# UoL-SignalProcessingGroup/SMC-NUTS

Hardware: NVIDIA B200
Metric: leapfrog_grad_evals_per_s (higher is better)
Workload: dtype f64

## Files before the change

### include/smcnuts_b200.h

```cpp
#ifndef SMCNUTS_B200_H
#define SMCNUTS_B200_H

#include <stdint.h>

#ifdef __cplusplus
extern "C" {
#endif

#define SMCB_MODEL_ARMA 0
#define SMCB_MODEL_PRMWCD 1
#define SMCB_MODEL_GAUSS 2

#define SMCB_STREAM_NUTS 0
#define SMCB_STREAM_MOMENTUM 1
#define SMCB_STREAM_ACCREJ 2
#define SMCB_STREAM_RESAMPLE 3
#define SMCB_STREAM_INIT 4
#define SMCB_STREAM_ESTIMATE 5

#define SMCB_CONSTRAIN_NONE 0
#define SMCB_CONSTRAIN_EXP_LAST 1

int smcb_version(void);
int smcb_build_flavour(void);
const char* smcb_last_error(void);
long long smcb_launch_count(void);

int smcb_model_create(int kind, const double* host_data, long long n, int dim, void** handle);
int smcb_model_create_plugin(const char* so_path, const double* host_data, long long n, void** handle);
int smcb_model_set_scale(void* handle, const double* host_scale);
int smcb_model_destroy(void* handle);
int smcb_model_dim(void* handle);
int smcb_model_constrained_dim(void* handle);
int smcb_model_constrain(void* handle, const double* x, long long N, double* out, void* stream);
int smcb_debug_pack_prm(const double* host_scalar_blob, int n_obs, int tiles, double* host_out, long long n_out);

int smcb_logp_grad(void* handle, const double* x, long long N, double phi, double* A, double* B, double* grad,
                   void* stream);
int smcb_combine_logp(const double* A, const double* B, double phi, long long N, double* out, void* stream);

int smcb_nuts_workspace_bytes(void* handle, long long N, int max_depth, long long* bytes);
int smcb_nuts_set_blocks_per_sm(int blocks_per_sm);
int smcb_nuts_transition(void* handle, const double* x, const double* r, long long N, double eps, double phi,
                         int max_depth, int accrej, uint64_t seed, uint32_t iteration, uint64_t particle0,
                         double* x_new, double* r_new, double* A_old, double* B_old, double* A_new, double* B_new,
                         double* ke_old, double* ke_new, int* n_leapfrog, int* accepted, int* depth, double* accept_stat,
                         const double* A_in, const double* B_in, const double* g_in, double* g_new, void* workspace,
                         long long workspace_bytes, void* stream);

int smcb_normals(uint64_t seed, uint32_t iteration, uint32_t stream_id, uint64_t particle0, long long N, int D,
                 double* out, void* stream);
int smcb_uniforms(uint64_t seed, uint32_t iteration, uint32_t stream_id, uint64_t particle0, long long N,
                  uint32_t draw, double* out, void* stream);

int smcb_row_half_sqnorm(const double* r, long long N, int D, double* out, void* stream);
int smcb_std_normal_logpdf(const double* x, long long N, int D, double* out, void* stream);
int smcb_uniform_logw(const double* logZ, long long N_total, long long N, double* out, void* stream);
int smcb_affine(const double* in, long long N, double a, double b, double* out, void* stream);
int smcb_init_logw(const double* lp, const double* x, long long N, int D, double* logw, void* stream);
int smcb_reweight_forward(const double* logw, const double* lp_x, const double* lp_xnew, const double* r,
                          const double* r_new, long long N, int D, double* out, void* stream);
int smcb_reweight_forward_ke(const double* logw, const double* lp_x, const double* lp_xnew, const double* ke_old,
                             const double* ke_new, long long N, double* out, void* stream);
int smcb_reweight_forward_split(const double* logw, const double* A_old, const double* B_old, const double* A_new,
                                const double* B_new, const double* ke_old, const double* ke_new, double phi, long long N,
                                double* out, void* stream);
int smcb_reweight_general(const double* logw, const double* lp_x, const double* lp_xnew, const double* L,
                          const double* q, long long N, double* out, void* stream);
int smcb_reweight_asymptotic(const double* logw, const double* A, const double* B, double phi_new, double phi_old,
                             long long N, double* out, void* stream);

long long smcb_reduce_workspace_bytes(void);
int smcb_lse_partial(const double* logw, long long N, double* out3, void* workspace, void* stream);
int smcb_lse_finalize(const double* triples, int P, double* out2, void* stream);
int smcb_normalise(const double* logw, long long N, const double* logZ, double* wn, void* stream);

int smcb_tempering_arrays(const double* A, const double* B, double phi_old, long long N, double* logpri,
                          double* loglik, double* c, void* stream);
int smcb_ess_multi_phi(const double* loglik, const double* logpri, const double* c, long long N,
                       const double* phis, int m, double* out, void* workspace, void* stream);

long long smcb_bisect_state_bytes(void);
int smcb_bisect_max_candidates(void);
int smcb_bisect_passes(void);
int smcb_bisect_init(void* state, double xa, double xb, double target, void* stream);
int smcb_bisect_eval(const double* A, const double* B, double phi_old, long long N, const void* state, double* out,
                     void* workspace, void* stream);
int smcb_bisect_step(const double* triples, int P, void* state, void* stream);
int smcb_bisect_read(const void* state, double* out4, void* stream);

long long smcb_scan_workspace_bytes(long long N);
int smcb_cdf(const double* wn, long long N, const double* offset_in, const double* total_in, double* cdf,
             double* total_out, void* workspace, void* stream);
int smcb_normalise_tilesums(const double* logw, long long N, const double* logZ, double* wn, double* total_out,
                            void* workspace, void* stream);
int smcb_cdf_from_tilesums(const double* wn, long long N, const double* offset_total, double* cdf, void* workspace,
                           void* stream);
int smcb_ancestors_multinomial(const double* cdf, long long N, const double* u, long long M, int64_t* idx,
                               void* stream);
int smcb_ancestors_systematic(const double* cdf, long long N, double u0, long long j0, long long M_total,
                              long long M, int64_t* idx, void* stream);
long long smcb_resample_workspace_bytes(long long M, int D);
int smcb_resample_systematic(const double* cdf, long long N, double u0, const double* u0_dev, long long j0,
                             long long M_total, long long M, const double* x, int D, double* out, int64_t* idx,
                             void* workspace, void* stream);
int smcb_resample_systematic_push(const double* cdf, long long N, double u0, long long j0, long long M_total,
                                  long long M, const double* x, int D, double* const* peer_out, long long rows_per_rank,
                                  int64_t* idx, void* workspace, void* stream);
int smcb_resample_multinomial_push(const double* cdf, long long n, const double* ends, int rank, int P, uint64_t seed,
                                   uint32_t iteration, uint32_t stream_id, long long N_total, long long particle0,
                                   const double* x, int D, double* const* peer_out, int64_t* const* peer_idx,
                                   long long rows_per_rank, void* stream);
int smcb_rank_offsets(const double* totals, int P, int rank, double* out2, void* stream);
int smcb_peer_alloc(long long bytes, void** ptr, void* handle64);
int smcb_peer_open(const void* handle64, void** ptr);
int smcb_peer_close(void* ptr);
int smcb_peer_free(void* ptr);
int smcb_gather_rows(const double* x, const int64_t* idx, long long M, int D, double* out, void* stream);

int smcb_scale_rows(const double* x, long long N, int D, const double* scale, int inverse, double* out, void* stream);

int smcb_weighted_moment(const double* x, const double* wn, long long N, int D, int constrain, const double* center,
                         int power, double* out, void* workspace, void* stream);
int smcb_weighted_moments12(const double* x, const double* wn, long long N, int D, int constrain, const double* center,
                            double* out2D, void* workspace, void* stream);
int smcb_moments12_finalize(const double* sums2D, const double* center, int D, double* mean, double* var, void* stream);
int smcb_count_moved(const double* x, const double* x_new, long long N, int D, double* out_count, void* workspace,
                     void* stream);

int smcb_gaussL_sums(const double* r_new, const double* x_new, long long N, int D, double* sums, void* stream);
int smcb_gaussL_gram(const double* r_new, const double* x_new, long long N, int D, const double* mean, double* gram,
// ... 23 lines not shown
```

### smc-nuts_b200/csrc/capi.cuh

```cuda
#pragma once
#include <cuda_runtime.h>

#include <atomic>
#include <cstdio>
#include <string>

#include "../../include/smcnuts_b200.h"
#include "common.cuh"
#include "models.cuh"

namespace smcb {

#if defined(SMCB_PLUGIN_TU)
inline std::string& last_error_ref() {
    static thread_local std::string s;
    return s;
}
inline std::atomic<long long> g_launches{0};
#else
std::string& last_error_ref();
extern std::atomic<long long> g_launches;
#endif

inline int fail(const char* where, const char* what) {
    last_error_ref() = std::string(where) + ": " + what;
    return -1;
}
inline int check_launch(const char* where) {
    g_launches.fetch_add(1, std::memory_order_relaxed);
    cudaError_t e = cudaGetLastError();
    if (e != cudaSuccess) return fail(where, cudaGetErrorString(e));
    return 0;
}
#define SMCB_CUDA(call)                                                        \
    do {                                                                       \
        cudaError_t e_ = (call);                                               \
        if (e_ != cudaSuccess) return ::smcb::fail(#call, cudaGetErrorString(e_)); \
    } while (0)
#define SMCB_REQUIRE(cond, msg)                          \
    do {                                                 \
        if (!(cond)) return ::smcb::fail(__func__, msg); \
    } while (0)

#define SMCB_PLUGIN_ABI 2
struct NutsArgs;
struct PluginVT {
    void* dl;
    int (*abi)(void);
    int (*dim)(void);
    int (*ndata)(void);
    const char* (*last_error)(void);
    long long (*nuts_workspace_bytes)(const ModelDesc*, long long, int);
    int (*nuts_transition)(const ModelDesc*, const NutsArgs*, long long, void*);
    int (*logp_grad)(const ModelDesc*, const double*, long long, double, double*, double*, double*, void*);
    int (*constrained_dim)(void);
    int (*constrain)(const ModelDesc*, const double*, long long, double*, void*);
};

struct Model {
    ModelDesc desc;
    double* d_data;
    PluginVT* vt = nullptr;
    double* d_scale = nullptr;
};

#if defined(SMCB_PLUGIN_TU)
inline int device_sm_count() {
    static int n = 0;
    if (!n) {
        int dev = 0;
        cudaGetDevice(&dev);
        cudaDeviceGetAttribute(&n, cudaDevAttrMultiProcessorCount, dev);
        if (n <= 0) n = 148;
    }
    return n;
}
#else
int device_sm_count();
#endif

inline int stride_grid(long long n, int threads, int per_sm) {
    long long want = (n + threads - 1) / threads;
    long long cap = (long long)device_sm_count() * per_sm;
    if (want < 1) want = 1;
    return (int)(want < cap ? want : cap);
}

}
```

### smc-nuts_b200/csrc/nuts_kernel.cu

```cuda
#include <dlfcn.h>

#include <cstdlib>
#include <cstring>
#include <vector>

#include "nuts_builtin.cuh"

namespace smcb {

std::string& last_error_ref() {
    static thread_local std::string s;
    return s;
}
std::atomic<long long> g_launches{0};
static thread_local int g_nuts_blocks_per_sm = 0;

int device_sm_count() {
    static int n = 0;
    if (!n) {
        int dev = 0;
        cudaGetDevice(&dev);
        cudaDeviceGetAttribute(&n, cudaDevAttrMultiProcessorCount, dev);
        if (n <= 0) n = 148;
    }
// ... 152 lines not shown
    if (N == 0) return 0;
    const Model* m = (const Model*)handle;
    if (m->vt->constrain(&m->desc, x, N, out, stream)) return fail("smcb_model_constrain (plug-in)", m->vt->last_error());
    g_launches.fetch_add(1, std::memory_order_relaxed);
    return 0;
}

int smcb_debug_pack_prm(const double* host_scalar_blob, int n_obs, int tiles, double* host_out, long long n_out) {
    SMCB_REQUIRE(host_scalar_blob && host_out && n_obs > 0 && tiles > 0 && n_obs <= 8 * tiles, "bad argument");
    SMCB_REQUIRE(n_out >= 32 + (long long)tiles * 9 * 32, "output too small: 32 + tiles * 288 doubles");
    pack_prm_fragments(host_scalar_blob, n_obs, tiles, host_out);
    return 0;
}

int smcb_logp_grad(void* handle, const double* x, long long N, double phi, double* A, double* B, double* grad,
                   void* stream) {
    SMCB_REQUIRE(handle && x && N >= 0, "bad argument");
    if (N == 0) return 0;
    const Model* m = (const Model*)handle;
    cudaStream_t st = (cudaStream_t)stream;
    if (m->vt) {
        if (m->vt->logp_grad(&m->desc, x, N, phi, A, B, grad, stream)) return fail("smcb_logp_grad (plug-in)", m->vt->last_error());
        g_launches.fetch_add(1, std::memory_order_relaxed);
        return 0;
    }
    switch (m->desc.kind) {
        case kArma: return launch_logp<ArmaModel>(m, x, N, phi, A, B, grad, st);
        case kPRMwCD: return launch_logp<PrmModel>(m, x, N, phi, A, B, grad, st);
        default: return launch_logp<GaussModel>(m, x, N, phi, A, B, grad, st);
    }
}

int smcb_combine_logp(const double* A, const double* B, double phi, long long N, double* out, void* stream) {
    SMCB_REQUIRE(A && B && out && N >= 0, "bad argument");
    if (N == 0) return 0;
    combine_logp_kernel<<<stride_grid(N, 256, 8), 256, 0, (cudaStream_t)stream>>>(A, B, phi, N, out);
    return check_launch("combine_logp_kernel");
}

int smcb_nuts_set_blocks_per_sm(int blocks_per_sm) {
    SMCB_REQUIRE(blocks_per_sm >= 0, "blocks_per_sm must be >= 0 (0 = as many as fit)");
    g_nuts_blocks_per_sm = blocks_per_sm;
    return 0;
}

int smcb_nuts_workspace_bytes(void* handle, long long N, int max_depth, long long* bytes) {
    SMCB_REQUIRE(handle && bytes && N >= 0, "bad argument");
    SMCB_REQUIRE(max_depth >= 1 && max_depth <= 10, "max_depth must be in [1, 10] (reference: MAX_TREE_DEPTH = 10)");
    const Model* m = (const Model*)handle;
    long long b;
    if (m->vt) {
        b = m->vt->nuts_workspace_bytes(&m->desc, N, max_depth);
        if (b < 0) return fail("smcb_nuts_workspace_bytes (plug-in)", "occupancy query failed");
        *bytes = b;
        return 0;
    }
    if (m->desc.scale) {
        b = nuts_ws_bytes_scaled(m, N, max_depth);
        if (b < 0) return fail("smcb_nuts_workspace_bytes", "occupancy query failed");
        *bytes = b;
        return 0;
    }
    switch (m->desc.kind) {
        case kArma: b = nuts_ws_bytes<ArmaModel>(m, N, max_depth); break;
        case kPRMwCD:
            b = prm_use_group(m->desc, N) ? nuts_ws_bytes<PrmModelG<kPrmTiles>>(m, N, max_depth) : nuts_ws_bytes<PrmModel>(m, N, max_depth);
            break;
        default: {
#define WS_G(K) nuts_ws_bytes<GaussModelG<K>>(m, N, max_depth)
            b = SMCB_GAUSS_DISPATCH(m->desc.dim, WS_G, nuts_ws_bytes<GaussModel>(m, N, max_depth));
#undef WS_G
            break;
        }
    }
    if (b < 0) return fail("smcb_nuts_workspace_bytes", "occupancy query failed");
    *bytes = b;
    return 0;
}

int smcb_nuts_transition(void* handle, const double* x, const double* r, long long N, double eps, double phi,
                         int max_depth, int accrej, uint64_t seed, uint32_t iteration, uint64_t particle0,
                         double* x_new, double* r_new, double* A_old, double* B_old, double* A_new, double* B_new,
                         double* ke_old, double* ke_new, int* n_leapfrog, int* accepted, int* depth, double* accept_stat,
                         const double* A_in, const double* B_in, const double* g_in, double* g_new, void* workspace,
                         long long workspace_bytes, void* stream) {
    SMCB_REQUIRE(handle && x && r && x_new && r_new && workspace, "null argument");
    SMCB_REQUIRE((A_in && B_in && g_in) || (!A_in && !B_in && !g_in), "A_in, B_in, g_in: all three or none");
    SMCB_REQUIRE(!(accrej && (g_in || g_new)), "gradient carry-over is not available with the accept-reject epilogue");
    SMCB_REQUIRE(g_new != x_new && (!g_in || (g_in != g_new)), "g_new must not alias its inputs");
    SMCB_REQUIRE(x != x_new && r != r_new, "x_new/r_new must not alias x/r");
    SMCB_REQUIRE(max_depth >= 1 && max_depth <= 10, "max_depth must be in [1, 10] (reference: MAX_TREE_DEPTH = 10)");
    SMCB_REQUIRE(iteration < (1u << 24), "iteration must be < 2^24");
    if (N <= 0) return N == 0 ? 0 : fail("smcb_nuts_transition", "negative N");
    const Model* m = (const Model*)handle;
    NutsArgs a{};
    a.model = m->desc;
    a.x = x; a.r = r; a.N = N; a.eps = eps; a.phi = phi; a.max_depth = max_depth; a.accrej = accrej;
    a.seed = seed; a.iteration = iteration; a.particle0 = particle0;
    a.x_new = x_new; a.r_new = r_new; a.A_old = A_old; a.B_old = B_old; a.A_new = A_new; a.B_new = B_new;
    a.ke_old = ke_old; a.ke_new = ke_new; a.n_leapfrog = n_leapfrog; a.accepted = accepted; a.depth = depth;
    a.accept_stat = accept_stat;
    a.blocks_per_sm = g_nuts_blocks_per_sm;
    a.A_in = A_in; a.B_in = B_in; a.g_in = g_in; a.g_new = g_new;
    a.ws = (double*)workspace;
    cudaStream_t st = (cudaStream_t)stream;
    if (m->vt) {
        if (m->vt->nuts_transition(&m->desc, &a, workspace_bytes, stream)) return fail("smcb_nuts_transition (plug-in)", m->vt->last_error());
        g_launches.fetch_add(1, std::memory_order_relaxed);
        return 0;
    }
    if (m->desc.scale) return launch_nuts_scaled(m, a, workspace_bytes, st);
    switch (m->desc.kind) {
        case kArma: return launch_nuts<ArmaModel>(m, a, workspace_bytes, st);
        case kPRMwCD:
            return prm_use_group(m->desc, N) ? launch_nuts<PrmModelG<kPrmTiles>>(m, a, workspace_bytes, st)
                                          : launch_nuts<PrmModel>(m, a, workspace_bytes, st);
        default: {
#define LAUNCH_G(K) launch_nuts<GaussModelG<K>>(m, a, workspace_bytes, st)
            return SMCB_GAUSS_DISPATCH(m->desc.dim, LAUNCH_G, launch_nuts<GaussModel>(m, a, workspace_bytes, st));
#undef LAUNCH_G
        }
    }
}

}
```

### smc-nuts_b200/csrc/nuts_lane.cuh

```cuda
#pragma once
#include "common.cuh"
#include "models.cuh"
#include "philox.cuh"

namespace smcb {

struct NutsArgs {
    ModelDesc model;
    const double* x;
    const double* r;
    long long N;
    double eps, phi;
    int max_depth;
    int accrej;
    uint64_t seed;
    uint32_t iteration;
    uint64_t particle0;
    double* x_new;
    double* r_new;
    double* A_old;
    double* B_old;
    double* A_new;
    double* B_new;
    double* ke_old;
    double* ke_new;
    int* n_leapfrog;
    int* accepted;
    int* depth;
    double* accept_stat;
    const double* A_in;
    const double* B_in;
    const double* g_in;
    double* g_new;
    double* ws;
    unsigned long long* queue;
    void* exchange;
    int blocks_per_sm;
};

struct alignas(16) D2 {
    double x, y;
};

SMCB_HD int nuts_nlp(int nl) { return (nl + 1) & ~1; }
SMCB_HD int nuts_stage_stride(int nl) { return 2 * nuts_nlp(nl) + 2; }
SMCB_HD int nuts_slot_stride(int nl, bool carry) { return 2 * nuts_nlp(nl) + 2 + (carry ? nuts_nlp(nl) : 0); }
constexpr int kNutsHdr = 8;
SMCB_HD int nuts_ws_doubles(int nl, int L, bool carry = true) {
    return ((kNutsHdr + 3 * nuts_nlp(nl) + nuts_slot_stride(nl, carry) * (2 * L + 3)) + 15) & ~15;
}

enum LanePhase : int { kIdle = 0, kInit = 1, kLeaf = 2 };

template <class M>
struct Lane {
    static constexpr int G = M::GROUP;
    static constexpr int DM = M::NLOC;
    double xa[DM], ra[DM], ga[DM];
    double logu;
    long long pid;
    double* ws;
    double* stg;
    int nlp_, slot_stride;
    int phase, dir, depth, D, L, nl, sub;
    uint32_t leaf, n_tot, n_leapfrog;
    uint32_t ck_used, cand_used, ck_valid;
    uint32_t samp_used;
    int samp_ref;
    uint64_t pend_n, pend_ref, ck_ref;
    StreamReader rng;

#define SMCB_LOCAL(i) for (int i = 0; i < (M::STATIC_NL ? M::STATIC_NL : nl); ++i)
#define SMCB_PAIRS(i) for (int i = 0; i < (M::STATIC_NL ? M::STATIC_NL : nl); i += 2)

    SMCB_HD int gd(int i) const { return G == 1 ? i : sub + G * i; }
    SMCB_HD uint64_t draw_bits(const NutsArgs& a) {
        return rng.next_bits(a.seed, (a.iteration << 8) | (uint32_t)kStreamNuts, a.particle0 + (uint64_t)pid);
    }
    SMCB_HD double draw(const NutsArgs& a) { return (double)draw_bits(a) * 0x1.0p-53; }
    SMCB_HD bool draw_below_ratio(const NutsArgs& a, uint32_t num, uint32_t den) {
        const uint64_t k = draw_bits(a);
        return k * (uint64_t)den < ((uint64_t)num << 53);
    }
    SMCB_HD int nlp_get() const { return M::STATIC_NL ? ((M::STATIC_NL + 1) & ~1) : nlp_; }
#define nlp nlp_get()
    SMCB_HD double gsum(double v) const {
#if defined(SMCB_WARP_CODE)
        if (G > 1) {
            const unsigned mask = ((1u << G) - 1u) << ((threadIdx.x & 31u) & ~(unsigned)(G - 1));
#pragma unroll
            for (int o = 1; o < G; o <<= 1) v += __shfl_xor_sync(mask, v, o);
        }
#endif
        return v;
    }

#ifndef SMCB_WIDE_RECORDS_CG
#define SMCB_WIDE_RECORDS_CG 1
#endif
    static constexpr bool kCg = (SMCB_WIDE_RECORDS_CG != 0) && M::STAGE;
// ... 488 lines not shown
```

### smc-nuts_b200/csrc/nuts_launch.cuh

```cuda
#pragma once
#include <cstdlib>

#include "capi.cuh"
#include "nuts_lane.cuh"

namespace smcb {

inline int blocks_per_sm_cap(int requested) {
    if (requested > 0) return requested;
    const char* e = getenv("SMCB_NUTS_BLOCKS_PER_SM");
    const int v = e ? atoi(e) : 0;
    return v > 0 ? v : 1 << 20;
}

template <class M> struct LaunchCfg { static constexpr int NT = 256, MIN_BLOCKS = 1; };

#ifndef SMCB_ALIGN_PARITY
#define SMCB_ALIGN_PARITY 0
#endif
template <class M> struct AlignCfg { static constexpr bool ON = (SMCB_ALIGN_PARITY != 0) && M::GROUP > 1; };

template <class M>
static size_t nuts_smem_bytes(const ModelDesc& d) {
    size_t n = (size_t)M::staged_doubles(d);
    if (M::STAGE) n += (size_t)LaunchCfg<M>::NT * nuts_stage_stride(M::STATIC_NL);
    return sizeof(double) * n;
}

template <class M> struct StageOffset { static int of(const ModelDesc&) { return 0; } };
template <class M> struct LaunchCfg<ScaledModel<M>> : LaunchCfg<M> {};
template <class M> struct StageOffset<ScaledModel<M>> : StageOffset<M> {};


template <class M>
__device__ __forceinline__ const double* stage_model(const ModelDesc& d, double* smem, int staged, int offset) {
    if constexpr (M::STATIC_NL != 0) {
        for (int i = threadIdx.x; i < staged; i += blockDim.x) smem[i] = d.data[offset + i];
        __syncthreads();
        return smem;
    } else {
        return d.data;
    }
}

#ifndef SMCB_TAIL_COMPACT
#define SMCB_TAIL_COMPACT 1
#endif
template <class M> struct TailCfg {
    static constexpr bool ON = (SMCB_TAIL_COMPACT != 0) && M::GROUP == 1 && !M::STAGE && !AlignCfg<M>::ON;
};

template <class M>
static size_t nuts_exchange_bytes(long long blocks) {
    return TailCfg<M>::ON ? (size_t)blocks * LaunchCfg<M>::NT * sizeof(Lane<M>) : 0;
}

template <class M>
__global__ void __launch_bounds__(LaunchCfg<M>::NT, LaunchCfg<M>::MIN_BLOCKS)
nuts_transition_kernel(NutsArgs a, int staged, int stage_offset, int rec_doubles) {
    extern __shared__ double smem[];
    constexpr int G = M::GROUP;
    constexpr int NW = LaunchCfg<M>::NT / 32;
    __shared__ int s_tail;
    __shared__ int s_cnt[2][NW];
    if (threadIdx.x == 0) s_tail = 0;
    M model(a.model, stage_model<M>(a.model, smem, staged, stage_offset));
    if constexpr (TailCfg<M>::ON) __syncthreads();
    const unsigned lane_id = threadIdx.x & 31u;
    Lane<M> lane;
    lane.idle_init(model, (int)(lane_id % G));
    lane.stg = M::STAGE ? smem + staged + (size_t)threadIdx.x * nuts_stage_stride(M::STATIC_NL) : nullptr;
    double* ws = a.ws + (size_t)(blockIdx.x * blockDim.x + threadIdx.x) * rec_doubles;
    constexpr unsigned kLeaders = G == 1 ? 0xffffffffu : 0x11111111u;
    const unsigned group_first = lane_id & ~(unsigned)(G - 1);
    bool drained = false;
    const unsigned admit_parity = a.g_in ? 1u : 0u;
    bool reported = false;
    for (unsigned trip = 0;; ++trip) {
        if constexpr (TailCfg<M>::ON) {
            if (*(volatile int*)&s_tail == NW) break;
        }
        const bool admit = !AlignCfg<M>::ON || ((trip & 1u) == admit_parity);
        const bool want = (lane.phase == kIdle) && !drained && admit;
        const unsigned m = __ballot_sync(0xffffffffu, want) & kLeaders;
        if (m) {
            const int leader = __ffs(m) - 1;
            unsigned long long base = 0;
            if ((int)lane_id == leader) base = atomicAdd(a.queue, (unsigned long long)__popc(m));
            base = __shfl_sync(0xffffffffu, base, leader);
            if (want) {
                const long long p = (long long)base + __popc(m & ((1u << group_first) - 1u));
                if (p < a.N) lane.begin(a, model, p, ws);
                else drained = true;
            }
            if constexpr (TailCfg<M>::ON) {
                if (!reported && __any_sync(0xffffffffu, drained)) {
                    if (lane_id == 0) atomicAdd(&s_tail, 1);
                    reported = true;
                }
            }
        }
        if (__all_sync(0xffffffffu, lane.phase == kIdle)) {
            if (!AlignCfg<M>::ON || __all_sync(0xffffffffu, drained)) break;
            continue;
        }
        if (lane.phase != kIdle) { lane.pre_eval(a); lane.prefetch_ck(); }
        double A, B, g[M::NLOC];
        if constexpr (G > 1) __syncwarp();
        model.eval(lane.xa, a.phi, A, B, g);
        lane.take_grad(g);
        if (lane.phase != kIdle) lane.post_eval(a, A, B);
    }
    if constexpr (TailCfg<M>::ON) {
        Lane<M>* exch = reinterpret_cast<Lane<M>*>(a.exchange) + (size_t)blockIdx.x * blockDim.x;
        const int warp = threadIdx.x >> 5;
        constexpr int kPerWarp = 32 / G;
        for (unsigned trip = 0;; ++trip) {
            const bool act = lane.phase != kIdle;
            const unsigned b = __ballot_sync(0xffffffffu, act) & kLeaders;
            if (lane_id == 0) s_cnt[trip & 1u][warp] = __popc(b);
            __syncthreads();
            int total = 0, before = 0, have = 0;
#pragma unroll
            for (int w = 0; w < NW; ++w) {
                const int c = s_cnt[trip & 1u][w];
                total += c;
                before += (w < warp) ? c : 0;
                have += (c > 0) ? 1 : 0;
            }
            if (total == 0) break;
            if (have > (total + kPerWarp - 1) / kPerWarp) {
                if (act) exch[(before + __popc(b & ((1u << group_first) - 1u))) * G + lane.sub] = lane;
                __threadfence();
                __syncthreads();
                if ((int)threadIdx.x < total * G) {
                    double* const stg = lane.stg;
                    lane = exch[threadIdx.x];
                    lane.stg = stg;
                } else {
                    lane.phase = kIdle;
                }
            }
            if (__all_sync(0xffffffffu, lane.phase == kIdle)) continue;
            if (lane.phase != kIdle) { lane.pre_eval(a); lane.prefetch_ck(); }
            double A, B, g[M::NLOC];
            if constexpr (G > 1) __syncwarp();
            model.eval(lane.xa, a.phi, A, B, g);
            lane.take_grad(g);
            if (lane.phase != kIdle) lane.post_eval(a, A, B);
        }
    }
}

template <class M>
__global__ void __launch_bounds__(128) logp_grad_kernel(ModelDesc md, const double* __restrict__ x, long long N,
                                                        double phi, double* __restrict__ Aout,
                                                        double* __restrict__ Bout, double* __restrict__ grad,
                                                        int staged) {
    extern __shared__ double smem[];
    M model(md, stage_model<M>(md, smem, staged, 0));
    const int D = M::STATIC_D ? M::STATIC_D : model.dim();
    for (long long i = blockIdx.x * (long long)blockDim.x + threadIdx.x; i < N; i += (long long)gridDim.x * blockDim.x) {
        double xv[M::DMAX], g[M::DMAX], A, B;
#pragma unroll
        for (int d = 0; d < (M::STATIC_D ? M::STATIC_D : D); ++d) xv[d] = x[i * D + d];
        model.eval(xv, phi, A, B, g);
        if (Aout) Aout[i] = A;
        if (Bout) Bout[i] = B;
        if (grad) {
            const bool bad = !is_finite(A + phi * B);
#pragma unroll
            for (int d = 0; d < (M::STATIC_D ? M::STATIC_D : D); ++d) grad[i * D + d] = bad ? neg_inf() : g[d];
        }
    }
}


template <class M>
static long long nuts_blocks(const Model* mdl, long long N, size_t smem, int* occ_out, int requested = 0) {
    const int NT = LaunchCfg<M>::NT;
    auto kern = nuts_transition_kernel<M>;
    if (smem > 48 * 1024) cudaFuncSetAttribute(kern, cudaFuncAttributeMaxDynamicSharedMemorySize, (int)smem);
    int occ = 0;
    if (cudaOccupancyMaxActiveBlocksPerMultiprocessor(&occ, kern, NT, smem) != cudaSuccess || occ < 1) return -1;
    if (occ > blocks_per_sm_cap(requested)) occ = blocks_per_sm_cap(requested);
    long long blocks = (long long)device_sm_count() * occ;
    const long long need = (N * M::GROUP + NT - 1) / NT;
    if (blocks > need) blocks = need;
    if (blocks < 1) blocks = 1;
    if (occ_out) *occ_out = occ;
    (void)mdl;
    return blocks;
}

template <class M>
static long long nuts_ws_bytes(const Model* mdl, long long N, int max_depth) {
    const size_t smem = nuts_smem_bytes<M>(mdl->desc);
    const long long blocks = nuts_blocks<M>(mdl, N, smem, nullptr);
    if (blocks < 0) return -1;
    M probe(mdl->desc, nullptr);
    return (long long)sizeof(double) * nuts_ws_doubles(probe.nloc(), max_depth) * blocks * LaunchCfg<M>::NT + 256 +
           (long long)nuts_exchange_bytes<M>(blocks);
}

template <class M>
static int launch_nuts(const Model* mdl, NutsArgs a, long long ws_bytes, cudaStream_t st) {
    const int NT = LaunchCfg<M>::NT;
    const int staged = M::staged_doubles(mdl->desc);
    const size_t smem = nuts_smem_bytes<M>(mdl->desc);
    const long long blocks = nuts_blocks<M>(mdl, a.N, smem, nullptr, a.blocks_per_sm);
    if (blocks < 0) return fail("smcb_nuts_transition", "kernel does not fit on an SM");
    M probe(mdl->desc, nullptr);
    const int rec = nuts_ws_doubles(probe.nloc(), a.max_depth, a.g_new != nullptr);
    const long long rec_bytes = (long long)sizeof(double) * rec * blocks * NT;
    const long long ws_need = rec_bytes + 256 + (long long)nuts_exchange_bytes<M>(blocks);
    if (ws_bytes < ws_need) return fail("smcb_nuts_transition", "workspace too small (see smcb_nuts_workspace_bytes)");
    a.queue = (unsigned long long*)((char*)a.ws + rec_bytes);
    a.exchange = (char*)a.ws + rec_bytes + 256;
    SMCB_CUDA(cudaMemsetAsync(a.queue, 0, sizeof(unsigned long long), st));
    nuts_transition_kernel<M><<<(int)blocks, NT, smem, st>>>(a, staged, StageOffset<M>::of(mdl->desc), rec);
    return check_launch("nuts_transition_kernel");
}


template <class M>
static int launch_logp(const Model* mdl, const double* x, long long N, double phi, double* A, double* B, double* g,
                       cudaStream_t st) {
    const int staged = M::staged_doubles(mdl->desc);
    const size_t smem = sizeof(double) * (size_t)staged;
    const int grid = stride_grid(N, 128, 8);
    logp_grad_kernel<M><<<grid, 128, smem, st>>>(mdl->desc, x, N, phi, A, B, g, staged);
    return check_launch("logp_grad_kernel");
}
// ... 3 lines not shown
```

### smc-nuts_b200/smcnuts/_cabi.py

```python
import ctypes
import re
from pathlib import Path

_PKG = Path(__file__).resolve().parent
import os
LIB_PATH = Path(os.environ.get("SMCB_LIB_PATH") or (_PKG / "_lib" / "libsmcnuts_b200.so"))
HEADER = _PKG.parents[1] / "include" / "smcnuts_b200.h"

MODEL_KINDS = {"arma": 0, "PRMwCD": 1, "gauss": 2}
STREAM_NUTS, STREAM_MOMENTUM, STREAM_ACCREJ, STREAM_RESAMPLE, STREAM_INIT, STREAM_ESTIMATE = range(6)
CONSTRAIN_NONE, CONSTRAIN_EXP_LAST = 0, 1
CONSTRAIN_MODEL = 2

_vp, _ll, _i, _d = ctypes.c_void_p, ctypes.c_longlong, ctypes.c_int, ctypes.c_double
_u64, _u32 = ctypes.c_uint64, ctypes.c_uint32

_SIGS = {
    "smcb_model_create": [_i, _vp, _ll, _i, ctypes.POINTER(_vp)],
    "smcb_model_create_plugin": [ctypes.c_char_p, _vp, _ll, ctypes.POINTER(_vp)],
    "smcb_model_set_scale": [_vp, _vp],
    "smcb_model_destroy": [_vp],
    "smcb_model_dim": [_vp],
    "smcb_model_constrained_dim": [_vp],
    "smcb_model_constrain": [_vp, _vp, _ll, _vp, _vp],
    "smcb_debug_pack_prm": [_vp, _i, _i, _vp, _ll],
    "smcb_logp_grad": [_vp, _vp, _ll, _d, _vp, _vp, _vp, _vp],
    "smcb_combine_logp": [_vp, _vp, _d, _ll, _vp, _vp],
    "smcb_nuts_workspace_bytes": [_vp, _ll, _i, ctypes.POINTER(_ll)],
    "smcb_nuts_set_blocks_per_sm": [_i],
    "smcb_nuts_transition": [_vp, _vp, _vp, _ll, _d, _d, _i, _i, _u64, _u32, _u64] + [_vp] * 16 + [_vp, _ll, _vp],
    "smcb_normals": [_u64, _u32, _u32, _u64, _ll, _i, _vp, _vp],
    "smcb_uniforms": [_u64, _u32, _u32, _u64, _ll, _u32, _vp, _vp],
    "smcb_row_half_sqnorm": [_vp, _ll, _i, _vp, _vp],
    "smcb_init_logw": [_vp, _vp, _ll, _i, _vp, _vp],
    "smcb_std_normal_logpdf": [_vp, _ll, _i, _vp, _vp],
    "smcb_uniform_logw": [_vp, _ll, _ll, _vp, _vp],
    "smcb_affine": [_vp, _ll, _d, _d, _vp, _vp],
    "smcb_reweight_forward": [_vp, _vp, _vp, _vp, _vp, _ll, _i, _vp, _vp],
    "smcb_reweight_forward_ke": [_vp, _vp, _vp, _vp, _vp, _ll, _vp, _vp],
    "smcb_reweight_forward_split": [_vp, _vp, _vp, _vp, _vp, _vp, _vp, _d, _ll, _vp, _vp],
    "smcb_reweight_general": [_vp, _vp, _vp, _vp, _vp, _ll, _vp, _vp],
    "smcb_reweight_asymptotic": [_vp, _vp, _vp, _d, _d, _ll, _vp, _vp],
    "smcb_lse_partial": [_vp, _ll, _vp, _vp, _vp],
    "smcb_lse_finalize": [_vp, _i, _vp, _vp],
    "smcb_normalise": [_vp, _ll, _vp, _vp, _vp],
    "smcb_tempering_arrays": [_vp, _vp, _d, _ll, _vp, _vp, _vp, _vp],
    "smcb_ess_multi_phi": [_vp, _vp, _vp, _ll, _vp, _i, _vp, _vp, _vp],
    "smcb_bisect_state_bytes": [],
    "smcb_bisect_max_candidates": [],
    "smcb_bisect_passes": [],
    "smcb_bisect_init": [_vp, _d, _d, _d, _vp],
    "smcb_bisect_eval": [_vp, _vp, _d, _ll, _vp, _vp, _vp, _vp],
    "smcb_bisect_step": [_vp, _i, _vp, _vp],
    "smcb_bisect_read": [_vp, _vp, _vp],
    "smcb_cdf": [_vp, _ll, _vp, _vp, _vp, _vp, _vp, _vp],
    "smcb_normalise_tilesums": [_vp, _ll, _vp, _vp, _vp, _vp, _vp],
    "smcb_cdf_from_tilesums": [_vp, _ll, _vp, _vp, _vp, _vp],
    "smcb_ancestors_multinomial": [_vp, _ll, _vp, _ll, _vp, _vp],
    "smcb_ancestors_systematic": [_vp, _ll, _d, _ll, _ll, _ll, _vp, _vp],
    "smcb_resample_systematic": [_vp, _ll, _d, _vp, _ll, _ll, _ll, _vp, _i, _vp, _vp, _vp, _vp],
    "smcb_resample_workspace_bytes": [_ll, _i],
    "smcb_resample_systematic_push": [_vp, _ll, _d, _ll, _ll, _ll, _vp, _i, _vp, _ll, _vp, _vp, _vp],
    "smcb_resample_multinomial_push": [_vp, _ll, _vp, _i, _i, _u64, _u32, _u32, _ll, _ll, _vp, _i, _vp, _vp, _ll, _vp],
    "smcb_rank_offsets": [_vp, _i, _i, _vp, _vp],
    "smcb_peer_alloc": [_ll, ctypes.POINTER(_vp), _vp],
    "smcb_peer_open": [_vp, ctypes.POINTER(_vp)],
    "smcb_peer_close": [_vp],
    "smcb_peer_free": [_vp],
    "smcb_gather_rows": [_vp, _vp, _ll, _i, _vp, _vp],
    "smcb_weighted_moment": [_vp, _vp, _ll, _i, _i, _vp, _i, _vp, _vp, _vp],
    "smcb_weighted_moments12": [_vp, _vp, _ll, _i, _i, _vp, _vp, _vp, _vp],
    "smcb_moments12_finalize": [_vp, _vp, _i, _vp, _vp, _vp],
    "smcb_count_moved": [_vp, _vp, _ll, _i, _vp, _vp, _vp],
    "smcb_gaussL_sums": [_vp, _vp, _ll, _i, _vp, _vp],
    "smcb_gaussL_gram": [_vp, _vp, _ll, _i, _vp, _vp, _vp],
    "smcb_gaussL_factor": [_vp, _ll, _i, _d, _vp, _vp, _vp, _vp],
    "smcb_gaussL_logpdf": [_vp, _vp, _ll, _i, _vp, _vp, _vp, _vp, _vp, _vp],
    "smcb_gaussL_logpdf_scratch_bytes": [_i],
    "smcb_sum_int32": [_vp, _ll, _vp, _vp, _vp],
    "smcb_sum_f64": [_vp, _ll, _vp, _vp, _vp],
    "smcb_scale_rows": [_vp, _ll, _i, _vp, _i, _vp, _vp],
    "smcb_fast_exp": [_vp, _ll, _vp, _vp],
    "smcb_fast_log": [_vp, _ll, _vp, _vp],
    "smcb_probe_fp64": [_i, _i, _i, _vp, _vp],
    "smcb_probe_dmma": [_i, _i, _i, _vp, _vp],
    "smcb_debug_dmma": [_vp, _vp, _vp, _vp, _i, _vp],
    "smcb_build_flavour": [],
    "smcb_version": [],
    "smcb_last_error": [],
    "smcb_launch_count": [],
    "smcb_reduce_workspace_bytes": [],
    "smcb_scan_workspace_bytes": [_ll],
}
_RESTYPES = {"smcb_last_error": ctypes.c_char_p, "smcb_launch_count": _ll, "smcb_reduce_workspace_bytes": _ll,
             "smcb_scan_workspace_bytes": _ll, "smcb_bisect_state_bytes": _ll, "smcb_resample_workspace_bytes": _ll,
             "smcb_gaussL_logpdf_scratch_bytes": _ll}

_LIB = None


class SmcbError(RuntimeError):
    pass


def declared_symbols():
    text = HEADER.read_text()
    return sorted(set(re.findall(r"\b(smcb_[a-zA-Z0-9_]+)\s*\(", text)))


def lib():
    global _LIB
    if _LIB is None:
        if not LIB_PATH.exists():
# ... 46 lines not shown
```

### smc-nuts_b200/smcnuts/proposal/nuts.py

```python

import os

import torch

from .. import _cabi, _device as dev

MAX_TREE_DEPTH = 10


def chunk_bounds(n, fractions):
    total, acc, bounds = sum(fractions), 0, [0]
    for c, f in enumerate(fractions):
        acc += f
        bounds.append(n if c + 1 == len(fractions) else max(bounds[-1], (acc * n) // total))
    return bounds


class NUTSProposal:
    accept_reject = False

    def __init__(self, target, momentum_proposal, step_size, rng=None, max_tree_depth=MAX_TREE_DEPTH):
        if not hasattr(target, "handle"):
            raise TypeError("the device NUTS proposal needs a device model (smcnuts.model.device_model / "
                            "smcnuts.model.bridgestan.StanModel); Python targets cannot run on the GPU path")
        self.target = target
        self.momentum_proposal = momentum_proposal
        self.step_size = float(step_size)
        self.rng = rng
        self.seed = dev.seed_from_rng(rng)
        self.max_tree_depth = int(max_tree_depth)
        self.iteration = 0
        self.particle0 = 0
        self.last = None
        self.record_events = False
        self.events = []
        self._ws_bytes = {}
        self.want_accept_stat = False

    PIPELINE_MIN_PARTICLES = 1 << 16
    PIPELINE_FRACTIONS = (1, 2, 3, 2, 1)
    PIPELINE_STREAMS = 4
    PIPELINE_BLOCKS_PER_SM = 0

    def rvs(self, x_cond, r_cond, phi: float = 1.0):
        D = self.target.dim
        host_in = dev.is_host(x_cond) or not x_cond.is_cuda
        n = (x_cond.size if dev.is_host(x_cond) else x_cond.numel()) // D if host_in else 0
        scaled = getattr(self.target, "_scale_dev", None) is not None
        if host_in and not scaled and n >= self.PIPELINE_MIN_PARTICLES and (dev.is_host(r_cond) or not r_cond.is_cuda):
            out = self._rvs_pipelined(x_cond, r_cond, float(phi), n)
            self.iteration += 1
            return out
        x = dev.to_device(x_cond).reshape(-1, D)
        r = dev.to_device(r_cond).reshape(-1, D)
        out = self.transition(x, r, phi)
        self.iteration += 1
        return dev.to_host_like(out["x_new"], x_cond, "x_new"), dev.to_host_like(out["r_new"], r_cond, "r_new")

    def _rvs_pipelined(self, x_cond, r_cond, phi, N):
        D = self.target.dim
        xh, x_pinned = dev.host_view(x_cond, N, D)
        rh, r_pinned = dev.host_view(r_cond, N, D)
        if not x_pinned:
            x_stage = dev.pinned_buffer("x_in", (N, D), torch.float64)
        if not r_pinned:
            r_stage = dev.pinned_buffer("r_in", (N, D), torch.float64)
        xo_h = dev.pinned_buffer("x_new", (N, D), torch.float64)
        ro_h = dev.pinned_buffer("r_new", (N, D), torch.float64)
        x, r = dev.empty(N, D), dev.empty(N, D)
        o = self._alloc_outputs(N, D, False)
        bounds = chunk_bounds(N, self.PIPELINE_FRACTIONS)
        nchunk = len(bounds) - 1
        nstream = min(self.PIPELINE_STREAMS, nchunk)
        streams = dev.side_streams(nstream)
        need = 0
        for lo, hi in zip(bounds, bounds[1:]):
            if hi > lo:
                nbytes = _cabi._ll()
                _cabi.call("smcb_nuts_workspace_bytes", self.target.handle, hi - lo, self.max_tree_depth, nbytes)
                need = max(need, nbytes.value)
        wss = [dev.workspace(f"nuts_pipe{i}", need) for i in range(nstream)]
        cur = torch.cuda.current_stream()
        ready = torch.cuda.Event()
        ready.record(cur)
        _cabi.call("smcb_nuts_set_blocks_per_sm", int(self.PIPELINE_BLOCKS_PER_SM))
        for c in range(nchunk):
            lo, hi = bounds[c], bounds[c + 1]
            if hi == lo:
                continue
            s = streams[c % nstream]
            if c < nstream:
                s.wait_event(ready)
            if not x_pinned:
                x_stage[lo:hi].copy_(xh[lo:hi])
            if not r_pinned:
                r_stage[lo:hi].copy_(rh[lo:hi])
            with torch.cuda.stream(s):
                x[lo:hi].copy_((xh if x_pinned else x_stage)[lo:hi], non_blocking=True)
                r[lo:hi].copy_((rh if r_pinned else r_stage)[lo:hi], non_blocking=True)
                self._launch(x, r, o, lo, hi, phi, self.iteration, None, wss[c % nstream], s.cuda_stream)
                xo_h[lo:hi].copy_(o["x_new"][lo:hi], non_blocking=True)
                ro_h[lo:hi].copy_(o["r_new"][lo:hi], non_blocking=True)
        _cabi.call("smcb_nuts_set_blocks_per_sm", 0)
        for s in streams:
            cur.wait_stream(s)
        cur.synchronize()
        self.last = o
        return dev.host_result(xo_h, x_cond), dev.host_result(ro_h, r_cond)

    def _workspace_bytes(self, N):
        key = (N, self.max_tree_depth, _cabi.LIB_PATH, os.environ.get("SMCB_PRM_SCALAR"), os.environ.get("SMCB_GAUSS_SCALAR"),
               os.environ.get("SMCB_NUTS_BLOCKS_PER_SM"), getattr(self.target, "_scale_dev", None) is not None)
        b = self._ws_bytes.get(key)
        if b is None:
            nbytes = _cabi._ll()
            _cabi.call("smcb_nuts_workspace_bytes", self.target.handle, N, self.max_tree_depth, nbytes)
            b = self._ws_bytes[key] = nbytes.value
        return b

    def _alloc_outputs(self, N, D, want_grad):
        o = dict(x_new=dev.empty(N, D), r_new=dev.empty(N, D), A_old=dev.empty(N), B_old=dev.empty(N),
                 A_new=dev.empty(N), B_new=dev.empty(N), ke_old=dev.empty(N), ke_new=dev.empty(N),
                 n_leapfrog=dev.empty(N, dtype=torch.int32), accepted=dev.empty(N, dtype=torch.int32),
                 depth=dev.empty(N, dtype=torch.int32))
        if want_grad:
            o["g_new"] = dev.empty(N, D)
        if self.want_accept_stat:
            o["accept_stat"] = dev.empty(N)
        return o

    def _launch(self, x, r, o, lo, hi, phi, it, carry, ws, stream):
        cA, cB, cg = carry if carry is not None else (None, None, None)
        sl = lambda t: dev.ptr(None if t is None else t[lo:hi])
        _cabi.call("smcb_nuts_transition", self.target.handle, sl(x), sl(r), hi - lo, self.step_size, float(phi),
                   self.max_tree_depth, int(self.accept_reject), self.seed, it, self.particle0 + lo,
                   sl(o["x_new"]), sl(o["r_new"]), sl(o["A_old"]), sl(o["B_old"]), sl(o["A_new"]), sl(o["B_new"]),
                   sl(o["ke_old"]), sl(o["ke_new"]), sl(o["n_leapfrog"]), sl(o["accepted"]), sl(o["depth"]),
                   sl(o.get("accept_stat")), sl(cA), sl(cB), sl(cg), sl(o.get("g_new")), dev.ptr(ws), ws.numel(), stream)

    def prepare(self, N, D, want_grad=False):
        want_grad = want_grad and not self.accept_reject
        self._prepared = ((N, D, want_grad, self.want_accept_stat), self._alloc_outputs(N, D, want_grad),
                          dev.workspace("nuts", self._workspace_bytes(N)))

    def transition(self, x, r, phi=1.0, iteration=None, carry=None, want_grad=False):
        N, D = x.shape
        it = self.iteration if iteration is None else iteration
        if self.accept_reject:
            carry, want_grad = None, False
        scale = getattr(self.target, "_scale_dev", None)
        if scale is not None:
            carry, want_grad = None, False
            z = dev.empty(N, D)
            _cabi.call("smcb_scale_rows", dev.ptr(x), N, D, dev.ptr(scale), 1, dev.ptr(z), dev.stream_ptr())
            x = z
        prepared, self._prepared = getattr(self, "_prepared", None), None
        if prepared is not None and prepared[0] == (N, D, want_grad, self.want_accept_stat):
            o, ws = prepared[1], prepared[2]
        else:
            o, ws = self._alloc_outputs(N, D, want_grad), dev.workspace("nuts", self._workspace_bytes(N))
        if self.record_events:
            e0, e1 = torch.cuda.Event(enable_timing=True), torch.cuda.Event(enable_timing=True)
            e0.record()
        self._launch(x, r, o, 0, N, phi, it, carry, ws, dev.stream_ptr())
        if self.record_events:
            e1.record()
            self.events.append((e0, e1))
        if scale is not None:
            _cabi.call("smcb_scale_rows", dev.ptr(o["x_new"]), N, D, dev.ptr(scale), 0, dev.ptr(o["x_new"]), dev.stream_ptr())
        self.last = o
        return o

    def logpdf(self, r):
        if dev.is_std_normal(self.momentum_proposal, self.target.dim):
            rd = dev.to_device(r).reshape(-1, self.target.dim)
            out = dev.empty(rd.shape[0])
            _cabi.call("smcb_std_normal_logpdf", dev.ptr(rd), rd.shape[0], self.target.dim, dev.ptr(out),
                       dev.stream_ptr())
            return dev.like_input(out, r)
        return self.momentum_proposal.logpdf(dev.to_numpy(r))
```

Measured before the change: 4.466 billion.

## Merge tail compaction into main NUTS loop and add optional particle order

Folds the block-level tail compaction loop into the main persistent work loop. Warps that finish admitting work switch into the exchange/compaction mode while others may still be admitting, instead of the block running a separate post-loop. It also adds an optional order permutation so the queue can admit particles in a caller-chosen order, for example longest trees first. The default order is null, so admission is unchanged unless a caller passes one; the plugin ABI version is bumped.

Result: slower. 4.319 billion, median of 6 (-3.3%).

```diff
diff --git a/include/smcnuts_b200.h b/include/smcnuts_b200.h
--- a/include/smcnuts_b200.h
+++ b/include/smcnuts_b200.h
@@ -45,8 +45,8 @@
                          int max_depth, int accrej, uint64_t seed, uint32_t iteration, uint64_t particle0,
                          double* x_new, double* r_new, double* A_old, double* B_old, double* A_new, double* B_new,
                          double* ke_old, double* ke_new, int* n_leapfrog, int* accepted, int* depth, double* accept_stat,
-                         const double* A_in, const double* B_in, const double* g_in, double* g_new, void* workspace,
-                         long long workspace_bytes, void* stream);
+                         const double* A_in, const double* B_in, const double* g_in, double* g_new, const int* order,
+                         void* workspace, long long workspace_bytes, void* stream);
 
 int smcb_normals(uint64_t seed, uint32_t iteration, uint32_t stream_id, uint64_t particle0, long long N, int D,
                  double* out, void* stream);
diff --git a/smc-nuts_b200/csrc/capi.cuh b/smc-nuts_b200/csrc/capi.cuh
--- a/smc-nuts_b200/csrc/capi.cuh
+++ b/smc-nuts_b200/csrc/capi.cuh
@@ -42,7 +42,7 @@
         if (!(cond)) return ::smcb::fail(__func__, msg); \
     } while (0)
 
-#define SMCB_PLUGIN_ABI 2
+#define SMCB_PLUGIN_ABI 3
 struct NutsArgs;
 struct PluginVT {
     void* dl;
diff --git a/smc-nuts_b200/csrc/nuts_kernel.cu b/smc-nuts_b200/csrc/nuts_kernel.cu
--- a/smc-nuts_b200/csrc/nuts_kernel.cu
+++ b/smc-nuts_b200/csrc/nuts_kernel.cu
@@ -258,8 +258,8 @@
                          int max_depth, int accrej, uint64_t seed, uint32_t iteration, uint64_t particle0,
                          double* x_new, double* r_new, double* A_old, double* B_old, double* A_new, double* B_new,
                          double* ke_old, double* ke_new, int* n_leapfrog, int* accepted, int* depth, double* accept_stat,
-                         const double* A_in, const double* B_in, const double* g_in, double* g_new, void* workspace,
-                         long long workspace_bytes, void* stream) {
+                         const double* A_in, const double* B_in, const double* g_in, double* g_new, const int* order,
+                         void* workspace, long long workspace_bytes, void* stream) {
     SMCB_REQUIRE(handle && x && r && x_new && r_new && workspace, "null argument");
     SMCB_REQUIRE((A_in && B_in && g_in) || (!A_in && !B_in && !g_in), "A_in, B_in, g_in: all three or none");
     SMCB_REQUIRE(!(accrej && (g_in || g_new)), "gradient carry-over is not available with the accept-reject epilogue");
@@ -272,7 +272,7 @@
     NutsArgs a{};
     a.model = m->desc;
     a.x = x; a.r = r; a.N = N; a.eps = eps; a.phi = phi; a.max_depth = max_depth; a.accrej = accrej;
-    a.seed = seed; a.iteration = iteration; a.particle0 = particle0;
+    a.seed = seed; a.iteration = iteration; a.particle0 = particle0; a.order = order;
     a.x_new = x_new; a.r_new = r_new; a.A_old = A_old; a.B_old = B_old; a.A_new = A_new; a.B_new = B_new;
     a.ke_old = ke_old; a.ke_new = ke_new; a.n_leapfrog = n_leapfrog; a.accepted = accepted; a.depth = depth;
     a.accept_stat = accept_stat;
diff --git a/smc-nuts_b200/csrc/nuts_lane.cuh b/smc-nuts_b200/csrc/nuts_lane.cuh
--- a/smc-nuts_b200/csrc/nuts_lane.cuh
+++ b/smc-nuts_b200/csrc/nuts_lane.cuh
@@ -16,6 +16,7 @@
     uint64_t seed;
     uint32_t iteration;
     uint64_t particle0;
+    const int* order;
     double* x_new;
     double* r_new;
     double* A_old;
diff --git a/smc-nuts_b200/csrc/nuts_launch.cuh b/smc-nuts_b200/csrc/nuts_launch.cuh
--- a/smc-nuts_b200/csrc/nuts_launch.cuh
+++ b/smc-nuts_b200/csrc/nuts_launch.cuh
@@ -76,33 +76,73 @@
     bool drained = false;
     const unsigned admit_parity = a.g_in ? 1u : 0u;
     bool reported = false;
+    bool tail = false;
+    unsigned tail_trip = 0;
+    Lane<M>* exch = reinterpret_cast<Lane<M>*>(a.exchange) + (size_t)blockIdx.x * blockDim.x;
     for (unsigned trip = 0;; ++trip) {
         if constexpr (TailCfg<M>::ON) {
-            if (*(volatile int*)&s_tail == NW) break;
-        }
-        const bool admit = !AlignCfg<M>::ON || ((trip & 1u) == admit_parity);
-        const bool want = (lane.phase == kIdle) && !drained && admit;
-        const unsigned m = __ballot_sync(0xffffffffu, want) & kLeaders;
-        if (m) {
-            const int leader = __ffs(m) - 1;
-            unsigned long long base = 0;
-            if ((int)lane_id == leader) base = atomicAdd(a.queue, (unsigned long long)__popc(m));
-            base = __shfl_sync(0xffffffffu, base, leader);
-            if (want) {
-                const long long p = (long long)base + __popc(m & ((1u << group_first) - 1u));
-                if (p < a.N) lane.begin(a, model, p, ws);
-                else drained = true;
+            if (!tail && *(volatile int*)&s_tail == NW) tail = true;
+        }
+        if (!tail) {
+            const bool admit = !AlignCfg<M>::ON || ((trip & 1u) == admit_parity);
+            const bool want = (lane.phase == kIdle) && !drained && admit;
+            const unsigned m = __ballot_sync(0xffffffffu, want) & kLeaders;
+            if (m) {
+                const int leader = __ffs(m) - 1;
+                unsigned long long base = 0;
+                if ((int)lane_id == leader) base = atomicAdd(a.queue, (unsigned long long)__popc(m));
+                base = __shfl_sync(0xffffffffu, base, leader);
+                if (want) {
+                    const long long p = (long long)base + __popc(m & ((1u << group_first) - 1u));
+                    if (p < a.N) lane.begin(a, model, a.order ? (long long)a.order[p] : p, ws);
+                    else drained = true;
+                }
+                if constexpr (TailCfg<M>::ON) {
+                    if (!reported && __any_sync(0xffffffffu, drained)) {
+                        if (lane_id == 0) atomicAdd(&s_tail, 1);
+                        reported = true;
+                    }
+                }
             }
-            if constexpr (TailCfg<M>::ON) {
-                if (!reported && __any_sync(0xffffffffu, drained)) {
-                    if (lane_id == 0) atomicAdd(&s_tail, 1);
-                    reported = true;
-                }
+            if (__all_sync(0xffffffffu, lane.phase == kIdle)) {
+                if (AlignCfg<M>::ON && !__all_sync(0xffffffffu, drained))
+                    continue;
+                if constexpr (!TailCfg<M>::ON) break;
+                tail = true;
             }
         }
-        if (__all_sync(0xffffffffu, lane.phase == kIdle)) {
-            if (!AlignCfg<M>::ON || __all_sync(0xffffffffu, drained)) break;
-            continue;
+        if constexpr (TailCfg<M>::ON) {
+            if (tail) {
+                const int warp = threadIdx.x >> 5;
+                constexpr int kPerWarp = 32 / G;
+                const unsigned par = tail_trip++ & 1u;
+                const bool act = lane.phase != kIdle;
+                const unsigned b = __ballot_sync(0xffffffffu, act) & kLeaders;
+                if (lane_id == 0) s_cnt[par][warp] = __popc(b);
+                __syncthreads();
+                int total = 0, before = 0, have = 0;
+#pragma unroll
+                for (int w = 0; w < NW; ++w) {
+                    const int c = s_cnt[par][w];
+                    total += c;
+                    before += (w < warp) ? c : 0;
+                    have += (c > 0) ? 1 : 0;
+                }
+                if (total == 0) break;
+                if (have > (total + kPerWarp - 1) / kPerWarp) {
+                    if (act) exch[(before + __popc(b & ((1u << group_first) - 1u))) * G + lane.sub] = lane;
+                    __threadfence();
+                    __syncthreads();
+                    if ((int)threadIdx.x < total * G) {
+                        double* const stg = lane.stg;
+                        lane = exch[threadIdx.x];
+                        lane.stg = stg;
+                    } else {
+                        lane.phase = kIdle;
+                    }
+                }
+                if (__all_sync(0xffffffffu, lane.phase == kIdle)) continue;
+            }
         }
         if (lane.phase != kIdle) { lane.pre_eval(a); lane.prefetch_ck(); }
         double A, B, g[M::NLOC];
@@ -110,45 +150,6 @@
         model.eval(lane.xa, a.phi, A, B, g);
         lane.take_grad(g);
         if (lane.phase != kIdle) lane.post_eval(a, A, B);
-    }
-    if constexpr (TailCfg<M>::ON) {
-        Lane<M>* exch = reinterpret_cast<Lane<M>*>(a.exchange) + (size_t)blockIdx.x * blockDim.x;
-        const int warp = threadIdx.x >> 5;
-        constexpr int kPerWarp = 32 / G;
-        for (unsigned trip = 0;; ++trip) {
-            const bool act = lane.phase != kIdle;
-            const unsigned b = __ballot_sync(0xffffffffu, act) & kLeaders;
-            if (lane_id == 0) s_cnt[trip & 1u][warp] = __popc(b);
-            __syncthreads();
-            int total = 0, before = 0, have = 0;
-#pragma unroll
-            for (int w = 0; w < NW; ++w) {
-                const int c = s_cnt[trip & 1u][w];
-                total += c;
-                before += (w < warp) ? c : 0;
-                have += (c > 0) ? 1 : 0;
-            }
-            if (total == 0) break;
-            if (have > (total + kPerWarp - 1) / kPerWarp) {
-                if (act) exch[(before + __popc(b & ((1u << group_first) - 1u))) * G + lane.sub] = lane;
-                __threadfence();
-                __syncthreads();
-                if ((int)threadIdx.x < total * G) {
-                    double* const stg = lane.stg;
-                    lane = exch[threadIdx.x];
-                    lane.stg = stg;
-                } else {
-                    lane.phase = kIdle;
-                }
-            }
-            if (__all_sync(0xffffffffu, lane.phase == kIdle)) continue;
-            if (lane.phase != kIdle) { lane.pre_eval(a); lane.prefetch_ck(); }
-            double A, B, g[M::NLOC];
-            if constexpr (G > 1) __syncwarp();
-            model.eval(lane.xa, a.phi, A, B, g);
-            lane.take_grad(g);
-            if (lane.phase != kIdle) lane.post_eval(a, A, B);
-        }
     }
 }
 
diff --git a/smc-nuts_b200/smcnuts/_cabi.py b/smc-nuts_b200/smcnuts/_cabi.py
--- a/smc-nuts_b200/smcnuts/_cabi.py
+++ b/smc-nuts_b200/smcnuts/_cabi.py
@@ -28,7 +28,7 @@
     "smcb_combine_logp": [_vp, _vp, _d, _ll, _vp, _vp],
     "smcb_nuts_workspace_bytes": [_vp, _ll, _i, ctypes.POINTER(_ll)],
     "smcb_nuts_set_blocks_per_sm": [_i],
-    "smcb_nuts_transition": [_vp, _vp, _vp, _ll, _d, _d, _i, _i, _u64, _u32, _u64] + [_vp] * 16 + [_vp, _ll, _vp],
+    "smcb_nuts_transition": [_vp, _vp, _vp, _ll, _d, _d, _i, _i, _u64, _u32, _u64] + [_vp] * 17 + [_vp, _ll, _vp],
     "smcb_normals": [_u64, _u32, _u32, _u64, _ll, _i, _vp, _vp],
     "smcb_uniforms": [_u64, _u32, _u32, _u64, _ll, _u32, _vp, _vp],
     "smcb_row_half_sqnorm": [_vp, _ll, _i, _vp, _vp],
diff --git a/smc-nuts_b200/smcnuts/proposal/nuts.py b/smc-nuts_b200/smcnuts/proposal/nuts.py
--- a/smc-nuts_b200/smcnuts/proposal/nuts.py
+++ b/smc-nuts_b200/smcnuts/proposal/nuts.py
@@ -98,7 +98,7 @@
             with torch.cuda.stream(s):
                 x[lo:hi].copy_((xh if x_pinned else x_stage)[lo:hi], non_blocking=True)
                 r[lo:hi].copy_((rh if r_pinned else r_stage)[lo:hi], non_blocking=True)
-                self._launch(x, r, o, lo, hi, phi, self.iteration, None, wss[c % nstream], s.cuda_stream)
+                self._launch(x, r, o, lo, hi, phi, self.iteration, None, None, wss[c % nstream], s.cuda_stream)
                 xo_h[lo:hi].copy_(o["x_new"][lo:hi], non_blocking=True)
                 ro_h[lo:hi].copy_(o["r_new"][lo:hi], non_blocking=True)
         _cabi.call("smcb_nuts_set_blocks_per_sm", 0)
@@ -129,21 +129,21 @@
             o["accept_stat"] = dev.empty(N)
         return o
 
-    def _launch(self, x, r, o, lo, hi, phi, it, carry, ws, stream):
+    def _launch(self, x, r, o, lo, hi, phi, it, carry, order, ws, stream):
         cA, cB, cg = carry if carry is not None else (None, None, None)
         sl = lambda t: dev.ptr(None if t is None else t[lo:hi])
         _cabi.call("smcb_nuts_transition", self.target.handle, sl(x), sl(r), hi - lo, self.step_size, float(phi),
                    self.max_tree_depth, int(self.accept_reject), self.seed, it, self.particle0 + lo,
                    sl(o["x_new"]), sl(o["r_new"]), sl(o["A_old"]), sl(o["B_old"]), sl(o["A_new"]), sl(o["B_new"]),
                    sl(o["ke_old"]), sl(o["ke_new"]), sl(o["n_leapfrog"]), sl(o["accepted"]), sl(o["depth"]),
-                   sl(o.get("accept_stat")), sl(cA), sl(cB), sl(cg), sl(o.get("g_new")), dev.ptr(ws), ws.numel(), stream)
+                   sl(o.get("accept_stat")), sl(cA), sl(cB), sl(cg), sl(o.get("g_new")), dev.ptr(order), dev.ptr(ws), ws.numel(), stream)
 
     def prepare(self, N, D, want_grad=False):
         want_grad = want_grad and not self.accept_reject
         self._prepared = ((N, D, want_grad, self.want_accept_stat), self._alloc_outputs(N, D, want_grad),
                           dev.workspace("nuts", self._workspace_bytes(N)))
 
-    def transition(self, x, r, phi=1.0, iteration=None, carry=None, want_grad=False):
+    def transition(self, x, r, phi=1.0, iteration=None, carry=None, want_grad=False, order=None):
         N, D = x.shape
         it = self.iteration if iteration is None else iteration
         if self.accept_reject:
@@ -162,7 +162,7 @@
         if self.record_events:
             e0, e1 = torch.cuda.Event(enable_timing=True), torch.cuda.Event(enable_timing=True)
             e0.record()
-        self._launch(x, r, o, 0, N, phi, it, carry, ws, dev.stream_ptr())
+        self._launch(x, r, o, 0, N, phi, it, carry, order, ws, dev.stream_ptr())
         if self.record_events:
             e1.record()
             self.events.append((e0, e1))
```
